# lukasmolnar/pino-locoman

Measured on AMD Instinct MI355X. Metric: MPC solves/sec (B2G whole_body_rnea N=50) at batch; 1/2/4/8 GPU, higher is better.
Workload: dtype f64; 1 GPU; b2g whole_body_rnea N=50 MPC step; batch_per_gpu=1024, global_batch=1024, nodes=50, robot=b2g, dynamics=whole_body_rnea, solver=osqp-sqp (1 SQP iteration, max_iter 100), parallelism=batch-sharded dp1

## Files before the change

include/pinoloco.h:

```cpp
#ifndef PINOLOCO_H_
#define PINOLOCO_H_

#ifdef __cplusplus
extern "C" {
#endif

typedef struct pl_model pl_model;
typedef struct pl_ocp pl_ocp;

#define PL_JOINT_FREEFLYER 1
#define PL_JOINT_REVOLUTE 2

#define PL_DYN_WHOLE_BODY_RNEA 0
#define PL_DYN_WHOLE_BODY_ACC 1
#define PL_DYN_WHOLE_BODY_ABA 2
#define PL_DYN_CENTROIDAL_VEL 3
#define PL_DYN_CENTROIDAL_ACC 4

typedef struct {
  int njoints;
  int nq, nv;
  const int* parent;
  const int* jtype;
  const double* axis;
// ... 194 lines not shown
int pl_dyn_jac_sizes(const pl_dyn* d, int fn, int flags, int* in_len, int* tan_len, int* out_len);
int pl_dyn_jac(pl_dyn* d, int fn, int batch, int frame, int flags, unsigned wrt, const double* in0,
               const double* in1, const double* in2, const double* in3, double* out, double* jac);
int pl_dyn_jac_device(pl_dyn* d, int fn, int batch, int frame, int flags, unsigned wrt, const void* in0,
                      const void* in1, const void* in2, const void* in3, void* out, void* jac);

#define PL_ADMM_AUTO 0
#define PL_ADMM_SWEEP 1
#define PL_ADMM_SWEEP2 2
#define PL_ADMM_CHAIN 3
int pl_ocp_set_admm_kernel(pl_ocp* o, int kind);
int pl_ocp_get_admm_kernel(const pl_ocp* o);
int pl_ocp_get_admm_groups(const pl_ocp* o);
#define PL_ADMM_OPERANDS_SPLIT 0
#define PL_ADMM_OPERANDS_FUSED 1
int pl_ocp_set_admm_operands(pl_ocp* o, int mode);
int pl_ocp_get_admm_operands(const pl_ocp* o);
int pl_ocp_get_admm_rho_from_bounds(const pl_ocp* o);

int pl_ocp_profile(pl_ocp* o, int enable);
int pl_ocp_profile_read(pl_ocp* o, double* out);
int pl_ocp_profile_read_hess(pl_ocp* o, double* out);
int pl_ocp_sizes(const pl_ocp* o, long long* out);

int pl_debug_get(pl_ocp* o, const char* name, double* out, long long count);
int pl_debug_set(pl_ocp* o, const char* name, const double* in, long long count);
int pl_debug_nodes(const pl_ocp* o, int* out);
int pl_debug_consts(const pl_ocp* o, void* model_out, void* oc_out, int* sizes);
int pl_debug_admm(pl_ocp* o, int niter, int reset);
int pl_debug_qp_setup(pl_ocp* o);
int pl_debug_check(pl_ocp* o, int final_check, int unscale);

#ifdef __cplusplus
}
#endif
#endif
```

pino-locoman_amd/csrc/api.hip:

```cpp
#include "api_internal.h"
#include "plant.h"
#include "record.h"
#include "retract.h"

#include <map>

static thread_local char g_err[1024] = "";

void pl_set_error(const char* fmt, ...) {
  va_list ap;
  va_start(ap, fmt);
  vsnprintf(g_err, sizeof(g_err), fmt, ap);
  va_end(ap);
}



extern "C" const char* pl_last_error(void) { return g_err; }
extern "C" int pl_version(void) { return 1; }

#ifndef PL_SRC_SHA
#define PL_SRC_SHA "unknown"
#endif
extern "C" const char* pl_build_info(void) { return "pl_src_sha256=" PL_SRC_SHA " arch=gfx950"; }
// ... 1658 lines not shown
  if (!out) { pl_set_error("null argument"); return -1; }
  prof_collect(&o->h);
  out[0] = o->h.prof_hess_ms;
  out[1] = (double)o->h.prof_hess_launches;
  int lanes = 0;
  if (o->h.d.ip_act)
    PL_CHECK_HIP(hipMemcpy(&lanes, o->h.d.ip_act + o->h.B + 1, sizeof(int), hipMemcpyDeviceToHost));
  out[2] = o->h.prof_hess_launches > 0 ? (double)lanes / o->h.prof_hess_launches : 0.0;
  return 0;
}

int admm_lds_bytes(const PlOcpHandle* h);
int admm_ppw(const PlOcpHandle* h);
int admm_asb_cap(const PlOcpHandle* h);

extern "C" int pl_ocp_sizes(const pl_ocp* o, long long* out) {
  if (!o) { pl_set_error("null handle"); return -1; }
  out[0] = o->h.n; out[1] = o->h.m; out[2] = o->h.nnz; out[3] = o->h.S_stride; out[4] = o->h.nw_max; out[5] = o->h.N;
  out[6] = (long long)o->aprog.size(); out[7] = admm_ppw(&o->h); out[8] = admm_lds_bytes(&o->h); out[9] = o->h.admm_asr;
  out[10] = admm_asb_cap(&o->h); out[11] = o->h.nent_max; out[12] = o->h.debug_paths;
  return 0;
}

static int debug_rw(pl_ocp* o, const char* name, double* out, const double* in, long long count) {
  PlOcpHandle* h = &o->h;
  const size_t B = h->B;
  struct Item { const char* n; double* p; size_t len; } items[] = {
      {"Hlag", h->d.Hlag, h->d.Hlag ? B * (size_t)h->hl_stride : 0},
      {"ip_dwi", h->d.ip_dwi, h->d.ip_dwi ? 2 * B : 0},
      {"As", h->d.As, B * h->nnz}, {"Araw", h->d.Araw, B * h->nnz}, {"qs", h->d.qs, B * h->n},
      {"ls", h->d.ls, B * h->m},   {"us", h->d.us, B * h->m},       {"rho", h->d.rho, B * h->m},
      {"D", h->d.D, B * h->n},     {"E", h->d.E, B * h->m},         {"cs", h->d.cs, B},
      {"admm_t", h->d.dbg, h->d.dbg ? B * 40 : 0}, {"Ps", h->d.Ps, B * h->n},   {"P", h->d.P, B * h->n},         {"xa", h->d.xa, B * h->n},
      {"za", h->d.za, B * h->m},   {"ya", h->d.ya, B * h->m},       {"S", h->d.S, B * (size_t)h->S_stride},
      {"FS", h->d.FS, h->d.FS ? B * (size_t)h->fs_stride : 0},
      {"rhs", h->d.rhs, B * h->n}, {"step", h->d.step, B * h->n},   {"grad", h->d.grad, B * h->n},
      {"g", h->d.g, B * h->m},     {"xstate", h->d.xstate, B * h->nx},
      {"dxs", h->d.dxs, B * h->n}, {"dys", h->d.dys, B * h->m},     {"chk", h->d.chk, B * (size_t)(h->N + 1) * 8},
      {"lbg", h->d.lbg, B * h->m}, {"ubg", h->d.ubg, B * h->m},
      {"rhoc", h->d.rhoc, B * (size_t)(h->N + 1) * std::max(h->ncpl_max, 1)},
      {"ip_s", h->d.ip_s, h->d.ip_s ? B * h->m : 0},     {"ip_lam", h->d.ip_lam, h->d.ip_lam ? B * h->m : 0},
      {"ip_lam0", h->d.ip_lam0, h->d.ip_lam0 ? B * h->m : 0},
      {"ip_zl", h->d.ip_zl, h->d.ip_zl ? B * h->m : 0},  {"ip_zu", h->d.ip_zu, h->d.ip_zu ? B * h->m : 0},
      {"ip_rh", h->d.ip_rh, h->d.ip_rh ? B * h->m : 0},  {"ip_dl", h->d.ip_dl, h->d.ip_dl ? B * h->m : 0},
      {"ip_ds", h->d.ip_ds, h->d.ip_ds ? B * h->m : 0},  {"ip_dx", h->d.ip_dx, h->d.ip_dx ? B * h->n : 0},
      {"ip_jdx", h->d.ip_jdx, h->d.ip_jdx ? B * h->m : 0}};
// ... 108 lines not shown
```

pino-locoman_amd/csrc/dyn_jac.h:

```cpp
#pragma once
#include "dyn.h"

namespace pl {

enum { PL_JF_NONE = -1, PL_JF_TREE = 0, PL_JF_COMP, PL_JF_ABA, PL_JF_CEN, PL_JF_FRAME, PL_JF_COUNT };

PL_HD int dyn_jac_family(int fn) {
  switch (fn) {
    case PL_FN_RNEA: case PL_FN_NLE: case PL_FN_GAPS_WB: return PL_JF_TREE;
    case PL_FN_GAPS_CA: case PL_FN_BASE_ACC_WB: case PL_FN_BASE_ACC_CV: return PL_JF_COMP;
    case PL_FN_ABA: return PL_JF_ABA;
    case PL_FN_COM_DYN: case PL_FN_GAPS_CV: case PL_FN_BASE_VEL_CV: case PL_FN_COM: return PL_JF_CEN;
    case PL_FN_FRAME_POS: case PL_FN_FRAME_VEL: return PL_JF_FRAME;
    default: return PL_JF_NONE;
  }
}
PL_HD int dyn_jac_cfg_input(int fn) { return (fn == PL_FN_BASE_VEL_CV || fn == PL_FN_GAPS_CV) ? 1 : 0; }
PL_HD void dyn_jac_tan_len(const PlModel& M, int fn, int nf, int* in_len, int* tan_len) {
  dyn_in_len(M, fn, nf, in_len);
  for (int k = 0; k < 4; ++k) tan_len[k] = in_len[k];
  tan_len[dyn_jac_cfg_input(fn)] = M.nv;
}
PL_HD void dyn_jac_locate(const int* tan_len, unsigned wrt, int col, int* input, int* local) {
  *input = -1;
// ... 107 lines not shown
    tree_pass<Dual>(M, O, qb, qr, SeedIn{in1, s1, 0}, SeedIn{nle ? nullptr : in2, s2, 0},
                    SeedIn{nle ? nullptr : in3, s3, 0}, true, false, kin);
    for (int r = 0; r < 6; ++r) out[r * ostride] = kin.tau[r].d;
    if (fn != PL_FN_GAPS_WB)
      for (int r = 6; r < nv; ++r) {
        const Dual t = kin.tau_j(r - 6);
        out[r * ostride] = t.d;
      }
  } else if constexpr (FAM == PL_JF_COMP) {
    Dual comp[15], res[6];
    const bool gap = fn == PL_FN_GAPS_CA;
    tree_pass<Dual>(M, O, qb, qr, SeedIn{in1, s1, 0}, SeedIn{in2, s2, gap ? 0 : 6}, SeedIn{in3, s3, 0}, true, false,
                    kin, comp, std::true_type{});
    if (gap) {
      centroidal_gap(M.total_mass, qb, comp, res);
    } else {
      Dual R0[9];
      quat_to_R(qb + 3, R0);
      base_solve(M.total_mass, R0, comp, kin.tau, res);
    }
    for (int r = 0; r < 6; ++r) out[r * ostride] = res[r].d;
  } else if constexpr (FAM == PL_JF_ABA) {
    tree_pass<Dual>(M, O, qb, qr, SeedIn{in1, s1, 0}, ShAcc{aba_sh}, SeedIn{in3, s3, 0}, true, false, kin);
    double* x = kin.dst + (PL_MAXV - 6 + 3 * PL_MAXFEET) * kin.dstride;
    for (int r = 0; r < 6; ++r) x[r * kin.dstride] = -kin.tau[r].d;
    for (int r = 0; r < nj; ++r) {
      const Dual t = kin.tau_j(r);
      x[(6 + r) * kin.dstride] = (r == s2 ? 1.0 : 0.0) - t.d;
    }
    chol_solve_strided(aba_sh + PL_MAXV, nv, x, kin.dstride);
    for (int r = 0; r < nv; ++r) out[r * ostride] = x[r * kin.dstride];
  } else if constexpr (FAM == PL_JF_CEN) {
    Dual hg[6], hd[6], ci[9];
    if (fn == PL_FN_COM_DYN) {
      centroidal_pass<Dual>(M, O, qb, qr, SeedIn{nullptr, -1, 0}, SeedIn{in1, s1, 0}, false, true, hg, hd);
      for (int r = 0; r < 6; ++r) out[r * ostride] = hd[r].d;
    } else if (fn == PL_FN_GAPS_CV) {
      centroidal_pass<Dual>(M, O, qb, qr, SeedIn{in2, s2, 0}, SeedIn{nullptr, -1, 0}, true, false, hg, hd);
      for (int r = 0; r < 6; ++r) out[r * ostride] = hg[r].d - (r == s0 ? M.total_mass : 0.0);
    } else if (fn == PL_FN_BASE_VEL_CV) {
      centroidal_pass<Dual>(M, O, qb, qr, SeedIn{in2, s2, 6}, SeedIn{nullptr, -1, 0}, true, false, hg, hd, ci,
                            std::true_type{});
      Dual R0[9], h[6], vb[6];
      quat_to_R(qb + 3, R0);
      for (int r = 0; r < 6; ++r) h[r] = Dual(in0[r], r == s0 ? 1.0 : 0.0);
      base_vel_solve(M.total_mass, R0, qb, ci, h, hg, vb);
      for (int r = 0; r < 6; ++r) out[r * ostride] = vb[r].d;
// ... 66 lines not shown
```

pino-locoman_amd/csrc/k_eval.hip:

```cpp
#include "dyn.h"
#include "eval_common.h"

using pl::VecIn;

namespace {

struct ValueEmit {
  double* g;
  double* lb;
  double* ub;
  int r;
  __device__ void operator()(double v, double l, double u) {
    g[r] = v;
    lb[r] = l;
    ub[r] = u;
    ++r;
  }
};

struct JacEmit {
  const int* rowidx;
  double* out;
  int ptr, end, r;
  __device__ void operator()(const Dual& v, double, double) {
// ... 23 lines not shown
template <int DYN>
__global__ __launch_bounds__(64) void k_eval_values(PlDev d, int B, int N, int n, int m, int np, const double* __restrict__ xsrc) {
  const int tid = blockIdx.x * blockDim.x + threadIdx.x;
  if (tid >= B * N) return;
  const int b = tid / N, i = tid - b * N;
  if (ip_skip(d, b)) return;
  const PlOcpConst& O = *d.oc;
  const PlModel& M = *d.model;
  const PlNode nd = d.nodes[i];
  const PlNode nn = d.nodes[i + 1];
  const double* x = xsrc + (size_t)b * n;
  const double* p = d.p + (size_t)b * np;
  VecIn<double> dx, u, dxn;
  node_inputs(d, nd, nn, x, nullptr, 0.0, -1, &dx, &u, &dxn, O.ndx);
  ValueEmit e{d.g + (size_t)b * m + nd.row_off, d.lbg + (size_t)b * m + nd.row_off,
              d.ubg + (size_t)b * m + nd.row_off, 0};
  __shared__ double kst[PL_KIN_STORE * 64];
  pl::node_rows<double, DYN>(M, O, i, p, dx, u, dxn, e, kst + threadIdx.x, 64);
}

#ifndef PL_JAC_WAVES
#define PL_JAC_WAVES 1
#endif
template <int DYN>
__global__ __launch_bounds__(64) __attribute__((amdgpu_waves_per_eu(PL_JAC_WAVES)))
void k_eval_jac(PlDev d, int B, int N, int n, int np, int nnz, int jl_len) {
  const int b = blockIdx.y;
  if (ip_skip(d, b)) return;
  const int q = (int)blockIdx.x * 64 + threadIdx.x;
  constexpr bool CH = DYN == PL_DYN_RNEA || DYN == PL_DYN_ACC;
  constexpr int SLOTS = CH ? PL_JAC_SLOTS_CH : PL_JAC_SLOTS;
  const int first = d.jlist[blockIdx.x * 64].x;
  const bool valid = q < jl_len && d.jlist[min(q, jl_len - 1)].x >= 0;
  const int2 jw = valid ? d.jlist[q] : make_int2(first, 0);
  const int i = jw.x, lc = jw.y & 0xffff, only_ch = CH ? (jw.y >> 16) - 1 : -1;
  const int slot = min(i - first, SLOTS - 1);
  __shared__ double kst_tan[PL_KIN_STORE_DUAL * 64];
  __shared__ double kst_val[SLOTS * PL_KIN_STORE_DUAL];
  double* aba_slot = nullptr;
  if constexpr (DYN == PL_DYN_ABA) {
    __shared__ double aba_sh[PL_JAC_SLOTS * PL_ABA_SH];
    aba_slot = aba_sh + slot * PL_ABA_SH;
    const int nv = d.oc->nv;
    double* raw = kst_tan + slot * ((PL_KIN_STORE_DUAL * 64) / PL_JAC_SLOTS);
    const bool tree = valid && lc < d.nodes[i].nw;
    int s0 = threadIdx.x, s1 = threadIdx.x;
    const int wb = (int)blockIdx.x * 64;
    if (tree) {
      while (s0 > 0 && d.jlist[wb + s0 - 1].x == i) --s0;
      while (s1 < 63 && wb + s1 + 1 < jl_len && d.jlist[wb + s1 + 1].x == i) ++s1;
    }
    const double* pb = d.p + (size_t)b * np;
    const double* dxi = d.x + (size_t)b * n + d.nodes[i].x_off;
    if (tree)
      for (int c = threadIdx.x - s0; c < nv + 2; c += s1 - s0 + 1) pl::aba_primal_column(*d.model, *d.oc, pb, dxi, c, raw + c * nv);
    __syncthreads();
    if (tree && threadIdx.x == s0) pl::aba_primal_finish(*d.oc, dxi, raw, aba_slot);
    __syncthreads();
  }
  if (!valid) return;
  const PlNode nd = d.nodes[i];
  const int* cp = d.colptr + nd.colptr_off;
  const int e0 = cp[lc], e1 = cp[lc + 1];
  const PlOcpConst& O = *d.oc;
  const PlModel& M = *d.model;
  const PlNode nn = d.nodes[i + 1];
  const double* x = d.x + (size_t)b * n;
  const double* p = d.p + (size_t)b * np;
  const int ndx = O.ndx;
  VecIn<Dual> dx{x + nd.x_off, nullptr, 0.0, lc};
  VecIn<Dual> u{x + nd.x_off + ndx, nullptr, 0.0, lc - ndx};
  VecIn<Dual> dxn{x + nn.x_off, nullptr, 0.0, lc - nd.nw};
  JacEmit e{d.rowidx + nd.ent_off, d.Araw + (size_t)b * nnz + nd.ent_off, e0, e1, 0};
  pl::node_rows<Dual, DYN>(M, O, i, p, dx, u, dxn, e, reinterpret_cast<Dual*>(kst_tan + threadIdx.x), 64,
                           kst_val + slot * PL_KIN_STORE_DUAL, aba_slot, nullptr, only_ch);
}

namespace {
struct ZeroInD {
  PL_HD double operator[](int) const { return 0.0; }
};
struct UnitIn {
  int k;
  PL_HD double operator[](int j) const { return j == k ? 1.0 : 0.0; }
};
}

template <int DYN>
__global__ __launch_bounds__(64) void k_eval_jac_lin(PlDev d, int B, int n, int np, int nnz, int len) {
  const int b = blockIdx.y;
  if (ip_skip(d, b)) return;
  const int q = (int)blockIdx.x * 64 + threadIdx.x;
  __shared__ double kst[PL_KIN_STORE * 64];
  __shared__ double kval[PL_KIN_STORE];
  for (int k = threadIdx.x; k < PL_KIN_STORE; k += 64) kval[k] = 0.0;
  __syncthreads();
  if (q >= len) return;
  const int2 jw = d.jlin[q];
// ... 4 lines not shown
  const PlNode nn = d.nodes[i + 1];
  const int ndx = O.ndx;
  const double* x = d.x + (size_t)b * n;
  const double* p = d.p + (size_t)b * np;
  const double* xi = p + O.P.x_init;
  const VecIn<double> dq{x + nd.x_off, nullptr, 0.0, -1};
  double qb[7];
  pl::integrate_ff<double>(xi, dq, qb);
  const pl::RevQ<double, VecIn<double>> qrev{xi, dq};
  pl::NodeKin<double> kp;
  kp.store = kst + threadIdx.x;
  kp.stride = 64;
  const int k = lc - ndx;
  pl::tree_pass<double>(*d.model0, O, qb, qrev, ZeroInD{}, UnitIn{k < O.na ? k : -1}, UnitIn{k - O.na}, true, false,
                        kp, nullptr, std::false_type{}, only_ch);
  double base[6];
  for (int r = 0; r < 6; ++r) base[r] = kp.tau[r];
  const int* cp = d.colptr + nd.colptr_off;
  VecIn<Dual> dx{x + nd.x_off, nullptr, 0.0, lc};
  VecIn<Dual> u{x + nd.x_off + ndx, nullptr, 0.0, lc - ndx};
  VecIn<Dual> dxn{x + nn.x_off, nullptr, 0.0, lc - nd.nw};
  JacEmit e{d.rowidx + nd.ent_off, d.Araw + (size_t)b * nnz + nd.ent_off, cp[lc], cp[lc + 1], 0};
  pl::node_rows<Dual, DYN>(*d.model, O, i, p, dx, u, dxn, e, reinterpret_cast<Dual*>(kst + threadIdx.x), 64, kval,
                           nullptr, base);
}

__global__ __launch_bounds__(256) void k_objective(PlDev d, int N, int n, int np) {
  const int b = blockIdx.x;
  if (ip_skip(d, b)) return;
  __shared__ double red[256];
  double f = objective_wg<true>(d, b, N, n, np, d.x + (size_t)b * n, nullptr, 0.0, d.grad + (size_t)b * n, red);
  if (threadIdx.x == 0) d.work[(size_t)b * 8 + 0] = f;
}

__global__ __launch_bounds__(256) void k_hess(PlDev d, int N, int n, int np) {
  const int b = blockIdx.x;
  const PlOcpConst& O = *d.oc;
  const double* p = d.p + (size_t)b * np;
  double* P = d.P + (size_t)b * n;
  for (int j = threadIdx.x; j < n; j += blockDim.x) {
    const int i = d.colnode[j];
    const int lc = j - d.nodes[i].x_off;
    double h;
    if (lc < O.ndx) {
      h = 2.0 * p[O.P.Q_diag + lc];
    } else {
      int k = lc - O.ndx;
// ... 3 lines not shown
    P[j] = h;
  }
}

#define PL_DISPATCH_DYN(dyn, KERNEL, ...)                                          \
  switch (dyn) {                                                                    \
    case PL_DYN_RNEA: hipLaunchKernelGGL(KERNEL<PL_DYN_RNEA>, __VA_ARGS__); break; \
    case PL_DYN_ACC: hipLaunchKernelGGL(KERNEL<PL_DYN_ACC>, __VA_ARGS__); break;   \
    case PL_DYN_CV: hipLaunchKernelGGL(KERNEL<PL_DYN_CV>, __VA_ARGS__); break;     \
    case PL_DYN_CA: hipLaunchKernelGGL(KERNEL<PL_DYN_CA>, __VA_ARGS__); break;     \
    case PL_DYN_ACCNB: hipLaunchKernelGGL(KERNEL<PL_DYN_ACCNB>, __VA_ARGS__); break; \
    case PL_DYN_CVNB: hipLaunchKernelGGL(KERNEL<PL_DYN_CVNB>, __VA_ARGS__); break;   \
    case PL_DYN_RNEAFD: hipLaunchKernelGGL(KERNEL<PL_DYN_RNEAFD>, __VA_ARGS__); break; \
    default: hipLaunchKernelGGL(KERNEL<PL_DYN_ABA>, __VA_ARGS__); break;           \
  }

void launch_eval_values(PlOcpHandle* h, const double* xsrc) {
  const int total = h->B * h->N;
  const int bs = 64;
  PL_DISPATCH_DYN(h->oc.dyn, k_eval_values, dim3((total + bs - 1) / bs), dim3(bs), 0, h->stream, h->d, h->B, h->N,
                  h->n, h->m, h->np, xsrc);
}

void launch_eval_jac(PlOcpHandle* h) {
  if (h->jlin_len > 0) {
    const dim3 g((h->jlin_len + 63) / 64, h->B);
    if (h->oc.dyn == PL_DYN_RNEA)
      hipLaunchKernelGGL(k_eval_jac_lin<PL_DYN_RNEA>, g, dim3(64), 0, h->stream, h->d, h->B, h->n, h->np, h->nnz,
                         h->jlin_len);
    else if (h->oc.dyn == PL_DYN_ACC)
      hipLaunchKernelGGL(k_eval_jac_lin<PL_DYN_ACC>, g, dim3(64), 0, h->stream, h->d, h->B, h->n, h->np, h->nnz,
                         h->jlin_len);
    else
      hipLaunchKernelGGL(k_eval_jac_lin<PL_DYN_RNEAFD>, g, dim3(64), 0, h->stream, h->d, h->B, h->n, h->np, h->nnz,
                         h->jlin_len);
  }
  const int len = (h->jac_cheap_ok && !h->jac_cheap_every) ? h->jl_ex : h->jl_len;
  if (len > 0)
    PL_DISPATCH_DYN(h->oc.dyn, k_eval_jac, dim3((len + 63) / 64, h->B), dim3(64), 0, h->stream, h->d, h->B, h->N,
                    h->n, h->np, h->nnz, h->jl_len);
  h->jac_cheap_ok = 1;
}

void launch_objective(PlOcpHandle* h) {
  hipLaunchKernelGGL(k_objective, dim3(h->B), dim3(256), 0, h->stream, h->d, h->N, h->n, h->np);
}

void launch_hess(PlOcpHandle* h) {
  hipLaunchKernelGGL(k_hess, dim3(h->B), dim3(256), 0, h->stream, h->d, h->N, h->n, h->np);
}

namespace {
struct ViolEmit {
  double ss, mx;
  __device__ void operator()(double v, double l, double u) {
    double a = fmax(0.0, l - v), c = fmax(0.0, v - u);
    ss += a * a + c * c;
    mx = fmax(mx, fmax(a, c));
  }
};

template <int DYN>
__device__ void violation_at(const PlDev& d, int b, int N, int n, int np, const double* x, const double* step,
                             double alpha, double* kst, double* red, double* metric, double* vmax) {
// ... 170 lines not shown
```

pino-locoman_amd/csrc/rbd.h:

```cpp
#pragma once
#include <type_traits>

#include "ad.h"
#include "model.h"

namespace pl {

template <class S> PL_HD void cross3(const S* a, const S* b, S* o) {
  S x = a[1] * b[2] - a[2] * b[1];
  S y = a[2] * b[0] - a[0] * b[2];
  S z = a[0] * b[1] - a[1] * b[0];
  o[0] = x; o[1] = y; o[2] = z;
}
template <class S> PL_HD S dot3(const S* a, const S* b) { return a[0] * b[0] + a[1] * b[1] + a[2] * b[2]; }
template <class S, class T, class X> PL_HD void matvec(const T* R, const X* x, S* o) {
  S a = R[0] * x[0] + R[1] * x[1] + R[2] * x[2];
  S b = R[3] * x[0] + R[4] * x[1] + R[5] * x[2];
  S c = R[6] * x[0] + R[7] * x[1] + R[8] * x[2];
  o[0] = a; o[1] = b; o[2] = c;
}
template <class S, class T, class X> PL_HD void mattvec(const T* R, const X* x, S* o) {
  S a = R[0] * x[0] + R[3] * x[1] + R[6] * x[2];
  S b = R[1] * x[0] + R[4] * x[1] + R[7] * x[2];
  S c = R[2] * x[0] + R[5] * x[1] + R[8] * x[2];
// ... 168 lines not shown
  S pxf[3];
  cross3(pp, fl, pxf);
  for (int k = 0; k < 3; ++k) { out[k] = fl[k]; out[3 + k] = nl[k] + pxf[k]; }
}
template <class S> PL_HD void inertia_mul(double m, const double* c, const double* Ic, const S* v, S* out) {
  S cc[3] = {S(c[0]), S(c[1]), S(c[2])};
  S cxw[3];
  cross3(cc, v + 3, cxw);
  S fl[3] = {m * (v[0] - cxw[0]), m * (v[1] - cxw[1]), m * (v[2] - cxw[2])};
  S Iw[3];
  matvec(Ic, v + 3, Iw);
  S cxf[3];
  cross3(cc, fl, cxf);
  for (int k = 0; k < 3; ++k) { out[k] = fl[k]; out[3 + k] = Iw[k] + cxf[k]; }
}
template <class S> PL_HD void motion_cross_force(const S* v, const S* f, S* out) {
  S a[3], b[3], c[3];
  cross3(v + 3, f, a);
  cross3(v + 3, f + 3, b);
  cross3(v, f, c);
  for (int k = 0; k < 3; ++k) { out[k] = a[k]; out[3 + k] = b[k] + c[k]; }
}

#define PL_KIN_STORE (PL_MAXV - 6 + 3 * PL_MAXFEET + 7 * PL_MAXCL)
#define PL_KIN_STORE_DUAL PL_KIN_STORE
#ifndef PL_CHAIN_UNROLL
#define PL_CHAIN_UNROLL 1
#endif
template <class S> struct NodeKin {
  S tau[6];
  S arm_vel[3];
  S* store;
  int stride;
  PL_HD S& tau_j(int k) { return store[k * stride]; }
  PL_HD S& foot_vel(int e, int c) { return store[(PL_MAXV - 6 + 3 * e + c) * stride]; }
  PL_HD S& sw(int kk, int c) { return store[(PL_MAXV - 6 + 3 * PL_MAXFEET + 7 * kk + c) * stride]; }
  PL_HD S& alpha(int kk) { return store[(PL_MAXV - 6 + 3 * PL_MAXFEET + 7 * kk + 6) * stride]; }
  PL_HD void clear(int k) { store[k * stride] = S(0.0); }
};

struct DualRef {
  double* v;
  double* d;
  PL_HD operator Dual() const { return Dual(*v, *d); }
  PL_HD DualRef& operator=(const Dual& x) {
    *v = x.v;
    *d = x.d;
    return *this;
  }
};
template <> struct NodeKin<Dual> {
  Dual tau[6];
  Dual arm_vel[3];
  double* vst;
  double* dst;
  int vstride, dstride;
  PL_HD DualRef at(int k) { return DualRef{vst + k * vstride, dst + k * dstride}; }
  PL_HD DualRef tau_j(int k) { return at(k); }
  PL_HD DualRef foot_vel(int e, int c) { return at(PL_MAXV - 6 + 3 * e + c); }
  PL_HD DualRef sw(int kk, int c) { return at(PL_MAXV - 6 + 3 * PL_MAXFEET + 7 * kk + c); }
  PL_HD DualRef alpha(int kk) { return at(PL_MAXV - 6 + 3 * PL_MAXFEET + 7 * kk + 6); }
  PL_HD void clear(int k) { dst[k * dstride] = 0.0; }
};

template <class S, class In> struct RevQ {
  const double* q0;
  In dq;
  PL_HD S operator()(int k) const { return q0[k] + dq[k - 1]; }
};
template <class S, class In> struct VelAcc {
  const double* v0;
  In dv;
  PL_HD S operator[](int k) const { return v0[k] + dv[k]; }
};
template <class S> struct RevQArr {
  const S* q;
  PL_HD S operator()(int k) const { return q[k]; }
};

template <class S>
PL_HD void comp_add(S* comp, double m, const double* lever, const double* Ic, const S* oR, const S* op, const S* p0) {
  S lw[3];
  matvec(oR, lever, lw);
  S r[3];
// ... 656 lines not shown
```

pino-locoman_amd/csrc/rows.h:

```cpp
#pragma once
#include <type_traits>

#include "rbd.h"

namespace pl {

PL_HD double spline_vel_z(double phase, double period, double h_max, double v_lo, double v_td) {
  double mid = period / 2.0;
  double t = phase * period;
  double t0, dt, c1, c2, c3;
  if (phase < 0.5) {
    t0 = 0.0; dt = mid - 0.0;
    double p0 = 0.0, v0 = v_lo, p1 = h_max, v1 = 0.0;
    double dpos = p1 - p0, dvel = v1 - v0;
    c1 = v0 * dt; c2 = -(3.0 * v0 + dvel) * dt + 3.0 * dpos; c3 = (2.0 * v0 + dvel) * dt - 2.0 * dpos;
  } else {
    t0 = mid; dt = period - mid;
    double p0 = h_max, v0 = 0.0, p1 = 0.0, v1 = v_td;
    double dpos = p1 - p0, dvel = v1 - v0;
    c1 = v0 * dt; c2 = -(3.0 * v0 + dvel) * dt + 3.0 * dpos; c3 = (2.0 * v0 + dvel) * dt - 2.0 * dpos;
  }
  double tn = (t - t0) / dt;
  return (3.0 * c3 * tn * tn + 2.0 * c2 * tn + c1) / dt;
}
// ... 71 lines not shown
PL_HD void chol_solve(const double* L, int n, double* x) {
  for (int i = 0; i < n; ++i) {
    const double* Li = L + i * (i + 1) / 2;
    double t = x[i];
    for (int k = 0; k < i; ++k) t -= Li[k] * x[k];
    x[i] = t / Li[i];
  }
  for (int i = n - 1; i >= 0; --i) {
    double t = x[i];
    for (int k = i + 1; k < n; ++k) t -= L[k * (k + 1) / 2 + i] * x[k];
    x[i] = t / L[i * (i + 1) / 2 + i];
  }
}

template <class E>
PL_HD auto emit_skip(E& e, int n, int) -> decltype(e.skip_block(n)) { return e.skip_block(n); }
template <class E>
PL_HD bool emit_skip(E&, int, long) { return false; }

template <class S, int DYN, class Emit>
PL_HD void node_rows(const PlModel& M, const PlOcpConst& O, int i, const double* p, const VecIn<S>& dx,
                     const VecIn<S>& u, const VecIn<S>& dxn, Emit& emit, S* kstore, int kstride,
                     double* kvals = nullptr, const double* aba_sh = nullptr, const double* lin_base = nullptr,
                     int only_ch = -1) {
  const int nv = O.nv, nq = O.nq, nj = O.nj;
  constexpr bool CV = PL_IS_CV(DYN);
  constexpr bool CVNB = (DYN == PL_DYN_CVNB);
  const double* xi = p + O.P.x_init;
  const double dt = node_dt(O, p, i);
  const int type = node_type(O, i);
  const double* xq = CV ? xi + 6 : xi;
  const VecIn<S> dq = CV ? sub_in(dx, 6) : dx;
  S qb[7];
  integrate_ff<S>(xq, dq, qb);
  const RevQ<S, VecIn<S>> qrev{xq, dq};
  S vnb[CVNB ? PL_MAXV : 1], hdot_nb[CVNB ? 6 : 1];
  if constexpr (CVNB) {
    bool run = true;
    if constexpr (!std::is_same<S, double>::value) run = !seeded(dxn, 0, O.ndx);
    if (run) {
      S hj[6], ci[9], hcur[6], R0[9];
      centroidal_pass<S>(M, O, qb, qrev, ZeroBaseAcc<S>{u}, sub_in(u, nj), true, true, hj, hdot_nb, ci,
                         std::true_type{});
      for (int k = 0; k < 6; ++k) hcur[k] = xi[k] + dx[k];
      quat_to_R(qb + 3, R0);
      base_vel_solve(M.total_mass, R0, qb, ci, hcur, hj, vnb);
    } else {
      for (int k = 0; k < 6; ++k) { vnb[k] = S(0.0); hdot_nb[k] = S(0.0); }
    }
    for (int k = 0; k < nj; ++k) vnb[6 + k] = u[k];
  }
  const auto vel = [&]() {
    if constexpr (CVNB) return static_cast<const S*>(vnb);
    else if constexpr (CV) return u;
    else return VelAcc<S, VecIn<S>>{xi + nq, sub_in(dx, nv)};
  }();
  constexpr bool ACCF = (DYN == PL_DYN_ACC || DYN == PL_DYN_CA || DYN == PL_DYN_ACCNB);
  constexpr bool NB = (DYN == PL_DYN_ACCNB);
  constexpr bool COMP = (DYN == PL_DYN_CA || DYN == PL_DYN_ACCNB);
  constexpr bool FD = (DYN == PL_DYN_RNEAFD);
  const int f_off = (PL_IS_RNEA(DYN) || ACCF) ? O.na : (DYN == PL_DYN_CV ? nv : nj);
  const VecIn<S> a = u;
  const FdAcc<S> afd{xi + nq, sub_in(dx, nv), sub_in(dxn, nv), dt};
  const VecIn<S> forces = sub_in(u, f_off);
  const VecIn<S> tau_j = sub_in(u, PL_IS_RNEA(DYN) ? O.na + O.nf : 0);
  const bool state_rows = CV || (type != 0);
  NodeKin<S> kin;
  if constexpr (std::is_same<S, Dual>::value) {
    double* raw = reinterpret_cast<double*>(kstore);
    if (kvals) {
      kin.vst = kvals;
      kin.vstride = 1;
      kin.dst = raw;
      kin.dstride = kstride;
    } else {
      kin.vst = raw;
      kin.dst = raw + 1;
      kin.vstride = kin.dstride = 2 * kstride;
    }
  } else {
    (void)kvals;
    kin.store = kstore;
    kin.stride = kstride;
  }
  constexpr bool want_tau = (PL_IS_RNEA(DYN) || ACCF);
  bool tree = true, cen = CV;
  if constexpr (!std::is_same<S, double>::value) {
    const bool seed_dxn = seeded(dxn, 0, FD ? nv : O.ndx);
    const bool seed_tau = PL_IS_RNEA(DYN) && seeded(u, O.na + O.nf, O.na + O.nf + nj);
    const bool seed_h = DYN == PL_DYN_CV && seeded(dx, 0, 6);
    const bool seed_f = CV && seeded(u, f_off, f_off + O.nf);
    const bool seed_pos = (PL_IS_RNEA(DYN) || DYN == PL_DYN_ACC) && seeded(dx, 0, 3);
    tree = !(seed_dxn || seed_tau || seed_h || seed_f || seed_pos) && !lin_base;
    cen = DYN == PL_DYN_CV && !(seed_dxn || seed_h);
  } else {
    (void)lin_base;
  }
  S comp[COMP ? 15 : 1];
  S aba_a[DYN == PL_DYN_ABA ? PL_MAXV : 1];
  bool aba_done = false;
  if constexpr (DYN == PL_DYN_ABA && std::is_same<S, Dual>::value) {
    {
      if (tree) {
        tree_pass<S>(M, O, qb, qrev, vel, ShAcc{aba_sh}, forces, true, state_rows, kin);
        double r[PL_MAXV];
        for (int k = 0; k < 6; ++k) r[k] = -kin.tau[k].d;
        for (int k = 0; k < nj; ++k) {
          const Dual t = kin.tau_j(k);
          r[6 + k] = tau_j[k].d - t.d;
        }
        chol_solve(aba_sh + PL_MAXV, nv, r);
        for (int k = 0; k < nv; ++k) aba_a[k] = Dual(aba_sh[k], r[k]);
      } else {
        for (int k = 0; k < PL_KIN_STORE_DUAL; ++k) kin.clear(k);
        for (int k = 0; k < 3; ++k) kin.arm_vel[k] = S(0.0);
        for (int k = 0; k < nv; ++k) aba_a[k] = S(0.0);
      }
      aba_done = true;
    }
  }
  if (aba_done) {
  } else if (tree && (want_tau || state_rows)) {
    if constexpr (NB) {
      tree_pass<S>(M, O, qb, qrev, vel, ZeroBaseAcc<S>{a}, forces, want_tau, state_rows, kin, comp, std::true_type{});
    } else if constexpr (COMP) {
      tree_pass<S>(M, O, qb, qrev, vel, a, forces, want_tau, state_rows, kin, comp, std::true_type{});
    } else if constexpr (FD) {
      tree_pass<S>(M, O, qb, qrev, vel, afd, forces, want_tau, state_rows, kin, nullptr, std::false_type{}, only_ch);
    } else {
      tree_pass<S>(M, O, qb, qrev, vel, a, forces, want_tau, state_rows, kin, nullptr, std::false_type{}, only_ch);
    }
  } else {
    for (int k = lin_base ? nj : 0; k < PL_KIN_STORE_DUAL; ++k) kin.clear(k);
    for (int k = 0; k < 3; ++k) kin.arm_vel[k] = S(0.0);
    for (int k = 0; k < 6; ++k) kin.tau[k] = S(0.0);
    if constexpr (COMP)
      for (int k = 0; k < 15; ++k) comp[k] = S(0.0);
    if constexpr (std::is_same<S, Dual>::value)
      if (lin_base)
        for (int k = 0; k < 6; ++k) kin.tau[k] = Dual(0.0, lin_base[k]);
  }
  S abase[NB ? 6 : 1], cgap[DYN == PL_DYN_CA ? 6 : 1];
  if constexpr (COMP) {
    if (tree) {
      S R0[9];
      quat_to_R(qb + 3, R0);
      if constexpr (NB) base_solve(M.total_mass, R0, comp, kin.tau, abase);
      else centroidal_gap(M.total_mass, qb, comp, cgap);
    } else {
      for (int k = 0; k < 6; ++k) {
        if constexpr (NB) abase[k] = S(0.0);
        else cgap[k] = S(0.0);
      }
    }
  }
  S hg[CV ? 6 : 1], hdot[CV ? 6 : 1];
// ... 111 lines not shown
```

pino-locoman_amd/pinoloco/_lib.py:

```python
from __future__ import annotations

import ctypes as C
import os

import numpy as np

HERE = os.path.dirname(os.path.abspath(__file__))
LIB_PATH = os.environ.get("PINOLOCO_LIB") or os.path.join(HERE, "libpinoloco.so")

_dp = C.POINTER(C.c_double)
_ip = C.POINTER(C.c_int)


class ModelDesc(C.Structure):
    _fields_ = [("njoints", C.c_int), ("nq", C.c_int), ("nv", C.c_int),
                ("parent", _ip), ("jtype", _ip), ("axis", _dp), ("placement_R", _dp), ("placement_p", _dp),
                ("mass", _dp), ("lever", _dp), ("inertia", _dp), ("gravity", _dp),
                ("nframes", C.c_int), ("frame_parent", _ip), ("frame_R", _dp), ("frame_p", _dp)]


class OcpDesc(C.Structure):
    _fields_ = [("dynamics", C.c_int), ("nodes", C.c_int), ("tau_nodes", C.c_int), ("include_acc", C.c_int),
                ("include_base", C.c_int), ("n_feet", C.c_int), ("foot_frames", C.c_int * 4),
                ("ext_force_frame", C.c_int), ("arm_ee_frame", C.c_int), ("base_frame", C.c_int),
# ... 93 lines not shown
    "pl_mpc_download": (C.c_int, [C.c_void_p, _dp]),
    "pl_ocp_retract_sizes": (C.c_int, [C.c_void_p, C.c_int, C.c_int, C.POINTER(C.c_longlong)]),
    "pl_ocp_retract": (C.c_int, [C.c_void_p, C.c_int, C.c_int, _dp, _dp, _dp, _dp, _dp, _dp]),
    "pl_ocp_retract_device": (C.c_int, [C.c_void_p, C.c_int, C.c_int, C.c_void_p]),
    "pl_ocp_profile_read_hess": (C.c_int, [C.c_void_p, _dp]),
    "pl_mpc_graph_info": (C.c_int, [C.c_void_p, C.POINTER(C.c_longlong)]),
    "pl_mpc_set_ip_lam": (C.c_int, [C.c_void_p, C.c_int]),
    "pl_mpc_log_start": (C.c_int, [C.c_void_p, C.c_longlong, C.c_int, _dp, _dp]),
    "pl_mpc_log_stop": (C.c_int, [C.c_void_p]),
    "pl_mpc_log_sizes": (C.c_int, [C.c_void_p, _llp]),
    "pl_mpc_log_read": (C.c_int, [C.c_void_p, C.c_longlong, C.c_longlong, _dp]),
    "pl_mpc_log_device": (C.c_int, [C.c_void_p, C.POINTER(C.c_void_p)]),
    "pl_mpc_metrics": (C.c_int, [C.c_void_p, C.POINTER(MpcMetrics)]),
    "pl_mpc_record_host": (C.c_int, [C.c_void_p, C.c_int, _dp, _dp, C.POINTER(Stats), _dp, _dp, _dp, C.c_double,
                                     _dp, _dp, _llp, _dp, C.POINTER(MpcMetrics)]),
    "pl_mpc_set_push": (C.c_int, [C.c_void_p, _ip, _ip, _dp]),
    "pl_mpc_run": (C.c_int, [C.c_void_p, C.c_int, C.c_int]),
    "pl_ocp_sync": (C.c_int, [C.c_void_p]),
    "pl_state_integrate": (C.c_int, [C.c_void_p, _dp, _dp, _dp]),
    "pl_state_difference": (C.c_int, [C.c_void_p, _dp, _dp, _dp]),
    "pl_ocp_profile": (C.c_int, [C.c_void_p, C.c_int]),
    "pl_ocp_profile_read": (C.c_int, [C.c_void_p, _dp]),
    "pl_ocp_sizes": (C.c_int, [C.c_void_p, C.POINTER(C.c_longlong)]),
    "pl_debug_consts": (C.c_int, [C.c_void_p, C.c_void_p, C.c_void_p, _ip]),
    "pl_debug_get": (C.c_int, [C.c_void_p, C.c_char_p, _dp, C.c_longlong]),
    "pl_debug_set": (C.c_int, [C.c_void_p, C.c_char_p, _dp, C.c_longlong]),
    "pl_debug_nodes": (C.c_int, [C.c_void_p, _ip]),
    "pl_debug_admm": (C.c_int, [C.c_void_p, C.c_int, C.c_int]),
    "pl_debug_qp_setup": (C.c_int, [C.c_void_p]),
    "pl_debug_check": (C.c_int, [C.c_void_p, C.c_int, C.c_int]),
    "pl_dyn_create": (C.c_int, [C.c_void_p, _ip, C.c_int, C.c_int, C.c_int, C.POINTER(C.c_void_p)]),
    "pl_dyn_destroy": (None, [C.c_void_p]),
    "pl_dyn_sizes": (C.c_int, [C.c_void_p, C.c_int, C.c_int, _ip, _ip]),
    "pl_dyn_eval": (C.c_int, [C.c_void_p, C.c_int, C.c_int, C.c_int, C.c_int, _dp, _dp, _dp, _dp, _dp]),
    "pl_dyn_jac_sizes": (C.c_int, [C.c_void_p, C.c_int, C.c_int, _ip, _ip, _ip]),
    "pl_dyn_jac": (C.c_int, [C.c_void_p, C.c_int, C.c_int, C.c_int, C.c_int, C.c_uint, _dp, _dp, _dp, _dp, _dp, _dp]),
    "pl_dyn_jac_device": (C.c_int, [C.c_void_p, C.c_int, C.c_int, C.c_int, C.c_int, C.c_uint, C.c_void_p, C.c_void_p,
                                    C.c_void_p, C.c_void_p, C.c_void_p, C.c_void_p]),
}

_lib = None


class PinolocoError(RuntimeError):
    pass

# ... 95 lines not shown
```

pino-locoman_amd/pinoloco/ocp.py:

```python
from __future__ import annotations

import ctypes as C
import time

import numpy as np

from . import _lib
from .dynamics import DYNAMICS_CLASSES, Dynamics
from .gait import horizon_dts

DYN_CODES = {"whole_body_rnea": 0, "whole_body_acc": 1, "whole_body_aba": 2, "centroidal_vel": 3,
             "centroidal_acc": 4}
GAIT_CODES = {"trot": 0, "walk": 1, "stand": 2}
SOLVER_CODES = {"osqp": 0, "fatrop": 1}

OSQP_SETTINGS = dict(max_iter=100, alpha=1.4, rho=2e-2, warm_start=True, adaptive_rho=False,
                     sigma=1e-6, eps_abs=1e-3, eps_rel=1e-3, eps_prim_inf=1e-4, eps_dual_inf=1e-4,
                     scaling=10, check_termination=25)

FATROP_SETTINGS = dict(max_iter=10, tol=1e-3, mu_init=1e-4, bound_push=1e-7, bound_frac=1e-2, delta_w=1e-8,
                       delta_c=1e-4, ls_max=12, n_refine=8, hessian=0)
IP_HESSIAN = {"exact": 0, "gauss_newton": 1}

OCP_ARGS = {
# ... 591 lines not shown
        return {"captures": int(out[0]), "replays": int(out[1]), "eager_fallback": int(out[2])}

    def sync(self):
        _lib.check(_lib.lib().pl_ocp_sync(self.h))

    def profile(self, enable):
        _lib.check(_lib.lib().pl_ocp_profile(self.h, int(enable)))

    def profile_read(self):
        out = np.zeros(3)
        _lib.check(_lib.lib().pl_ocp_profile_read(self.h, _lib.dptr(out)))
        return {"admm_ms": out[0], "launches": int(out[1]), "problem_iters": int(out[2])}

    def profile_read_hess(self):
        out = np.zeros(3)
        _lib.check(_lib.lib().pl_ocp_profile_read_hess(self.h, _lib.dptr(out)))
        return {"hess_ms": out[0], "launches": int(out[1]), "lanes": out[2]}

    def sizes(self):
        out = (C.c_longlong * 13)()
        _lib.check(_lib.lib().pl_ocp_sizes(self.h, out))
        return dict(zip(("n", "m", "nnz", "S_stride", "nw_max", "N", "admm_prog", "admm_ppw", "admm_lds_bytes",
                         "admm_asr", "admm_asb_cap", "nent_max", "debug_paths"), [int(v) for v in out]))

    def close(self):
        if getattr(self, "h", None):
            _lib.lib().pl_ocp_destroy(self.h)
            self.h = None

    def __del__(self):
        try:
            self.close()
        except Exception:
            pass


class ModelCache:
    _cache = {}

    @classmethod
    def get(cls, model):
        key = id(model)
        if key not in cls._cache:
            cls._cache[key] = (model, _lib.ModelHandle(model))
        return cls._cache[key][1]

# ... 382 lines not shown
```

Measured before the change: 10210 solves/s.

## Shrink k_eval_jac LDS footprint via dynamic shared memory and scratch sink layout

Reorders the kinematic store so foot-velocity and contact scratch come first and tau last. The Jacobian kernel's value store now keeps only the per-slot non-scratch part and sends output values to a shared sink. For RNEA/ACC the LDS is allocated dynamically, sized by the model's actual joint count instead of PL_MAXV. The smaller LDS use is meant to allow more resident waves per CU. It also adds an API to report LDS sizes, and the index remapping risks subtle aliasing bugs.

```diff
diff --git a/include/pinoloco.h b/include/pinoloco.h
--- a/include/pinoloco.h
+++ b/include/pinoloco.h
@@ -240,6 +240,8 @@
 int pl_ocp_profile_read(pl_ocp* o, double* out);
 int pl_ocp_profile_read_hess(pl_ocp* o, double* out);
 int pl_ocp_sizes(const pl_ocp* o, long long* out);
+#define PL_LDS_SIZES_LEN 50
+int pl_ocp_lds_sizes(const pl_ocp* o, long long* out);
 
 int pl_debug_get(pl_ocp* o, const char* name, double* out, long long count);
 int pl_debug_set(pl_ocp* o, const char* name, const double* in, long long count);
diff --git a/pino-locoman_amd/csrc/api.hip b/pino-locoman_amd/csrc/api.hip
--- a/pino-locoman_amd/csrc/api.hip
+++ b/pino-locoman_amd/csrc/api.hip
@@ -1704,6 +1704,23 @@
   return 0;
 }
 
+int eval_jac_lds_bytes(const PlOcpHandle* h, int* out);
+
+extern "C" int pl_ocp_lds_sizes(const pl_ocp* o, long long* out) {
+  if (!o || !out) { pl_set_error("null argument"); return -1; }
+  int jac = 0;
+  if (eval_jac_lds_bytes(&o->h, &jac) != 0) { pl_set_error("hipFuncGetAttributes(k_eval_jac) failed"); return -1; }
+  out[0] = jac;
+  out[1] = o->h.nfgroup;
+  for (int g = 0; g < PL_FAC_MAXGROUPS; ++g) {
+    const bool on = g < o->h.nfgroup;
+    out[2 + 3 * g] = on ? o->h.fg_i0[g] : 0;
+    out[3 + 3 * g] = on ? o->h.fg_n[g] : 0;
+    out[4 + 3 * g] = on ? o->h.fg_lds[g] : 0;
+  }
+  return 0;
+}
+
 static int debug_rw(pl_ocp* o, const char* name, double* out, const double* in, long long count) {
   PlOcpHandle* h = &o->h;
   const size_t B = h->B;
diff --git a/pino-locoman_amd/csrc/dyn_jac.h b/pino-locoman_amd/csrc/dyn_jac.h
--- a/pino-locoman_amd/csrc/dyn_jac.h
+++ b/pino-locoman_amd/csrc/dyn_jac.h
@@ -153,7 +153,7 @@
     for (int r = 0; r < 6; ++r) out[r * ostride] = res[r].d;
   } else if constexpr (FAM == PL_JF_ABA) {
     tree_pass<Dual>(M, O, qb, qr, SeedIn{in1, s1, 0}, ShAcc{aba_sh}, SeedIn{in3, s3, 0}, true, false, kin);
-    double* x = kin.dst + (PL_MAXV - 6 + 3 * PL_MAXFEET) * kin.dstride;
+    double* x = kin.dst + PL_KIN_SCR * kin.dstride;
     for (int r = 0; r < 6; ++r) x[r * kin.dstride] = -kin.tau[r].d;
     for (int r = 0; r < nj; ++r) {
       const Dual t = kin.tau_j(r);
diff --git a/pino-locoman_amd/csrc/k_eval.hip b/pino-locoman_amd/csrc/k_eval.hip
--- a/pino-locoman_amd/csrc/k_eval.hip
+++ b/pino-locoman_amd/csrc/k_eval.hip
@@ -69,6 +69,14 @@
 #ifndef PL_JAC_WAVES
 #define PL_JAC_WAVES 1
 #endif
+#define PL_JAC_LDS_BUDGET 40960
+constexpr int jac_val_doubles(int slots) { return (slots * PL_KIN_NSCR + 2) & ~1; }
+constexpr int jac_lds_bytes(int slots, int nj) { return (jac_val_doubles(slots) + (PL_KIN_TAU + nj) * 64) * 8; }
+static_assert(jac_lds_bytes(PL_JAC_SLOTS_CH, 18) <= PL_JAC_LDS_BUDGET,
+              "k_eval_jac<RNEA / ACC>: a wave of an 18-joint model must fit a quarter of the CU's LDS");
+static_assert(jac_lds_bytes(PL_JAC_SLOTS, PL_MAXV - 6) <= PL_JAC_LDS_BUDGET,
+              "k_eval_jac, three-slot instantiations: the store must fit a quarter of the CU's LDS");
+extern __shared__ double jac_dyn_lds[];
 template <int DYN>
 __global__ __launch_bounds__(64) __attribute__((amdgpu_waves_per_eu(PL_JAC_WAVES)))
 void k_eval_jac(PlDev d, int B, int N, int n, int np, int nnz, int jl_len) {
@@ -82,8 +90,16 @@
   const int2 jw = valid ? d.jlist[q] : make_int2(first, 0);
   const int i = jw.x, lc = jw.y & 0xffff, only_ch = CH ? (jw.y >> 16) - 1 : -1;
   const int slot = min(i - first, SLOTS - 1);
-  __shared__ double kst_tan[PL_KIN_STORE_DUAL * 64];
-  __shared__ double kst_val[SLOTS * PL_KIN_STORE_DUAL];
+  double *kst_tan, *kst_val;
+  if constexpr (CH) {
+    kst_val = jac_dyn_lds;
+    kst_tan = jac_dyn_lds + jac_val_doubles(SLOTS);
+  } else {
+    __shared__ double tan_st[PL_KIN_STORE_DUAL * 64];
+    __shared__ double val_st[jac_val_doubles(SLOTS)];
+    kst_tan = tan_st;
+    kst_val = val_st;
+  }
   double* aba_slot = nullptr;
   if constexpr (DYN == PL_DYN_ABA) {
     __shared__ double aba_sh[PL_JAC_SLOTS * PL_ABA_SH];
@@ -120,7 +136,7 @@
   VecIn<Dual> dxn{x + nn.x_off, nullptr, 0.0, lc - nd.nw};
   JacEmit e{d.rowidx + nd.ent_off, d.Araw + (size_t)b * nnz + nd.ent_off, e0, e1, 0};
   pl::node_rows<Dual, DYN>(M, O, i, p, dx, u, dxn, e, reinterpret_cast<Dual*>(kst_tan + threadIdx.x), 64,
-                           kst_val + slot * PL_KIN_STORE_DUAL, aba_slot, nullptr, only_ch);
+                           kst_val + slot * PL_KIN_NSCR, aba_slot, nullptr, only_ch, kst_val + SLOTS * PL_KIN_NSCR);
 }
 
 namespace {
@@ -171,7 +187,7 @@
   VecIn<Dual> dxn{x + nn.x_off, nullptr, 0.0, lc - nd.nw};
   JacEmit e{d.rowidx + nd.ent_off, d.Araw + (size_t)b * nnz + nd.ent_off, cp[lc], cp[lc + 1], 0};
   pl::node_rows<Dual, DYN>(*d.model, O, i, p, dx, u, dxn, e, reinterpret_cast<Dual*>(kst + threadIdx.x), 64, kval,
-                           nullptr, base);
+                           nullptr, base, -1, kval + PL_KIN_NSCR);
 }
 
 __global__ __launch_bounds__(256) void k_objective(PlDev d, int N, int n, int np) {
@@ -221,6 +237,11 @@
                   h->n, h->m, h->np, xsrc);
 }
 
+static int jac_dynamic_lds(const PlOcpHandle* h) {
+  const bool ch = h->oc.dyn == PL_DYN_RNEA || h->oc.dyn == PL_DYN_ACC;
+  return ch ? jac_lds_bytes(PL_JAC_SLOTS_CH, h->oc.nj) : 0;
+}
+
 void launch_eval_jac(PlOcpHandle* h) {
   if (h->jlin_len > 0) {
     const dim3 g((h->jlin_len + 63) / 64, h->B);
@@ -236,9 +257,27 @@
   }
   const int len = (h->jac_cheap_ok && !h->jac_cheap_every) ? h->jl_ex : h->jl_len;
   if (len > 0)
-    PL_DISPATCH_DYN(h->oc.dyn, k_eval_jac, dim3((len + 63) / 64, h->B), dim3(64), 0, h->stream, h->d, h->B, h->N,
-                    h->n, h->np, h->nnz, h->jl_len);
+    PL_DISPATCH_DYN(h->oc.dyn, k_eval_jac, dim3((len + 63) / 64, h->B), dim3(64), jac_dynamic_lds(h), h->stream, h->d,
+                    h->B, h->N, h->n, h->np, h->nnz, h->jl_len);
   h->jac_cheap_ok = 1;
+}
+
+int eval_jac_lds_bytes(const PlOcpHandle* h, int* out) {
+  hipFuncAttributes a;
+  hipError_t e;
+  switch (h->oc.dyn) {
+    case PL_DYN_RNEA: e = hipFuncGetAttributes(&a, reinterpret_cast<const void*>(&k_eval_jac<PL_DYN_RNEA>)); break;
+    case PL_DYN_ACC: e = hipFuncGetAttributes(&a, reinterpret_cast<const void*>(&k_eval_jac<PL_DYN_ACC>)); break;
+    case PL_DYN_CV: e = hipFuncGetAttributes(&a, reinterpret_cast<const void*>(&k_eval_jac<PL_DYN_CV>)); break;
+    case PL_DYN_CA: e = hipFuncGetAttributes(&a, reinterpret_cast<const void*>(&k_eval_jac<PL_DYN_CA>)); break;
+    case PL_DYN_ACCNB: e = hipFuncGetAttributes(&a, reinterpret_cast<const void*>(&k_eval_jac<PL_DYN_ACCNB>)); break;
+    case PL_DYN_CVNB: e = hipFuncGetAttributes(&a, reinterpret_cast<const void*>(&k_eval_jac<PL_DYN_CVNB>)); break;
+    case PL_DYN_RNEAFD: e = hipFuncGetAttributes(&a, reinterpret_cast<const void*>(&k_eval_jac<PL_DYN_RNEAFD>)); break;
+    default: e = hipFuncGetAttributes(&a, reinterpret_cast<const void*>(&k_eval_jac<PL_DYN_ABA>)); break;
+  }
+  if (e != hipSuccess) return -1;
+  *out = (int)a.sharedSizeBytes + jac_dynamic_lds(h);
+  return 0;
 }
 
 void launch_objective(PlOcpHandle* h) {
diff --git a/pino-locoman_amd/csrc/rbd.h b/pino-locoman_amd/csrc/rbd.h
--- a/pino-locoman_amd/csrc/rbd.h
+++ b/pino-locoman_amd/csrc/rbd.h
@@ -214,7 +214,10 @@
   for (int k = 0; k < 3; ++k) { out[k] = a[k]; out[3 + k] = b[k] + c[k]; }
 }
 
-#define PL_KIN_STORE (PL_MAXV - 6 + 3 * PL_MAXFEET + 7 * PL_MAXCL)
+#define PL_KIN_SCR (3 * PL_MAXFEET)
+#define PL_KIN_NSCR (7 * PL_MAXCL)
+#define PL_KIN_TAU (PL_KIN_SCR + PL_KIN_NSCR)
+#define PL_KIN_STORE (PL_KIN_TAU + PL_MAXV - 6)
 #define PL_KIN_STORE_DUAL PL_KIN_STORE
 #ifndef PL_CHAIN_UNROLL
 #define PL_CHAIN_UNROLL 1
@@ -224,10 +227,10 @@
   S arm_vel[3];
   S* store;
   int stride;
-  PL_HD S& tau_j(int k) { return store[k * stride]; }
-  PL_HD S& foot_vel(int e, int c) { return store[(PL_MAXV - 6 + 3 * e + c) * stride]; }
-  PL_HD S& sw(int kk, int c) { return store[(PL_MAXV - 6 + 3 * PL_MAXFEET + 7 * kk + c) * stride]; }
-  PL_HD S& alpha(int kk) { return store[(PL_MAXV - 6 + 3 * PL_MAXFEET + 7 * kk + 6) * stride]; }
+  PL_HD S& tau_j(int k) { return store[(PL_KIN_TAU + k) * stride]; }
+  PL_HD S& foot_vel(int e, int c) { return store[(3 * e + c) * stride]; }
+  PL_HD S& sw(int kk, int c) { return store[(PL_KIN_SCR + 7 * kk + c) * stride]; }
+  PL_HD S& alpha(int kk) { return store[(PL_KIN_SCR + 7 * kk + 6) * stride]; }
   PL_HD void clear(int k) { store[k * stride] = S(0.0); }
 };
 
@@ -247,11 +250,23 @@
   double* vst;
   double* dst;
   int vstride, dstride;
-  PL_HD DualRef at(int k) { return DualRef{vst + k * vstride, dst + k * dstride}; }
-  PL_HD DualRef tau_j(int k) { return at(k); }
-  PL_HD DualRef foot_vel(int e, int c) { return at(PL_MAXV - 6 + 3 * e + c); }
-  PL_HD DualRef sw(int kk, int c) { return at(PL_MAXV - 6 + 3 * PL_MAXFEET + 7 * kk + c); }
-  PL_HD DualRef alpha(int kk) { return at(PL_MAXV - 6 + 3 * PL_MAXFEET + 7 * kk + 6); }
+  int omask = -1, soff = 0;
+  PL_HD void bind_scratch(double* scr, double* sink, double* d, int ds) {
+    vst = sink;
+    vstride = 1;
+    omask = 0;
+    soff = (int)(scr - sink) - PL_KIN_SCR;
+    dst = d;
+    dstride = ds;
+  }
+  PL_HD DualRef out_at(int k) { return DualRef{vst + (k & omask) * vstride, dst + k * dstride}; }
+  PL_HD DualRef scr_at(int k) {
+    return DualRef{vst + ((PL_KIN_SCR + k) * vstride + soff), dst + (PL_KIN_SCR + k) * dstride};
+  }
+  PL_HD DualRef tau_j(int k) { return out_at(PL_KIN_TAU + k); }
+  PL_HD DualRef foot_vel(int e, int c) { return out_at(3 * e + c); }
+  PL_HD DualRef sw(int kk, int c) { return scr_at(7 * kk + c); }
+  PL_HD DualRef alpha(int kk) { return scr_at(7 * kk + 6); }
   PL_HD void clear(int k) { dst[k * dstride] = 0.0; }
 };
 
diff --git a/pino-locoman_amd/csrc/rows.h b/pino-locoman_amd/csrc/rows.h
--- a/pino-locoman_amd/csrc/rows.h
+++ b/pino-locoman_amd/csrc/rows.h
@@ -117,7 +117,7 @@
 PL_HD void node_rows(const PlModel& M, const PlOcpConst& O, int i, const double* p, const VecIn<S>& dx,
                      const VecIn<S>& u, const VecIn<S>& dxn, Emit& emit, S* kstore, int kstride,
                      double* kvals = nullptr, const double* aba_sh = nullptr, const double* lin_base = nullptr,
-                     int only_ch = -1) {
+                     int only_ch = -1, double* ksink = nullptr) {
   const int nv = O.nv, nq = O.nq, nj = O.nj;
   constexpr bool CV = PL_IS_CV(DYN);
   constexpr bool CVNB = (DYN == PL_DYN_CVNB);
@@ -164,10 +164,7 @@
   if constexpr (std::is_same<S, Dual>::value) {
     double* raw = reinterpret_cast<double*>(kstore);
     if (kvals) {
-      kin.vst = kvals;
-      kin.vstride = 1;
-      kin.dst = raw;
-      kin.dstride = kstride;
+      kin.bind_scratch(kvals, ksink, raw, kstride);
     } else {
       kin.vst = raw;
       kin.dst = raw + 1;
@@ -207,7 +204,7 @@
         chol_solve(aba_sh + PL_MAXV, nv, r);
         for (int k = 0; k < nv; ++k) aba_a[k] = Dual(aba_sh[k], r[k]);
       } else {
-        for (int k = 0; k < PL_KIN_STORE_DUAL; ++k) kin.clear(k);
+        for (int k = 0; k < PL_KIN_TAU + nj; ++k) kin.clear(k);
         for (int k = 0; k < 3; ++k) kin.arm_vel[k] = S(0.0);
         for (int k = 0; k < nv; ++k) aba_a[k] = S(0.0);
       }
@@ -226,7 +223,7 @@
       tree_pass<S>(M, O, qb, qrev, vel, a, forces, want_tau, state_rows, kin, nullptr, std::false_type{}, only_ch);
     }
   } else {
-    for (int k = lin_base ? nj : 0; k < PL_KIN_STORE_DUAL; ++k) kin.clear(k);
+    for (int k = 0; k < (lin_base ? PL_KIN_TAU : PL_KIN_TAU + nj); ++k) kin.clear(k);
     for (int k = 0; k < 3; ++k) kin.arm_vel[k] = S(0.0);
     for (int k = 0; k < 6; ++k) kin.tau[k] = S(0.0);
     if constexpr (COMP)
diff --git a/pino-locoman_amd/pinoloco/_lib.py b/pino-locoman_amd/pinoloco/_lib.py
--- a/pino-locoman_amd/pinoloco/_lib.py
+++ b/pino-locoman_amd/pinoloco/_lib.py
@@ -139,6 +139,7 @@
     "pl_ocp_profile": (C.c_int, [C.c_void_p, C.c_int]),
     "pl_ocp_profile_read": (C.c_int, [C.c_void_p, _dp]),
     "pl_ocp_sizes": (C.c_int, [C.c_void_p, C.POINTER(C.c_longlong)]),
+    "pl_ocp_lds_sizes": (C.c_int, [C.c_void_p, C.POINTER(C.c_longlong)]),
     "pl_debug_consts": (C.c_int, [C.c_void_p, C.c_void_p, C.c_void_p, _ip]),
     "pl_debug_get": (C.c_int, [C.c_void_p, C.c_char_p, _dp, C.c_longlong]),
     "pl_debug_set": (C.c_int, [C.c_void_p, C.c_char_p, _dp, C.c_longlong]),
diff --git a/pino-locoman_amd/pinoloco/ocp.py b/pino-locoman_amd/pinoloco/ocp.py
--- a/pino-locoman_amd/pinoloco/ocp.py
+++ b/pino-locoman_amd/pinoloco/ocp.py
@@ -637,6 +637,12 @@
         _lib.check(_lib.lib().pl_ocp_sizes(self.h, out))
         return dict(zip(("n", "m", "nnz", "S_stride", "nw_max", "N", "admm_prog", "admm_ppw", "admm_lds_bytes",
                          "admm_asr", "admm_asb_cap", "nent_max", "debug_paths"), [int(v) for v in out]))
+
+    def lds_sizes(self):
+        out = (C.c_longlong * 50)()
+        _lib.check(_lib.lib().pl_ocp_lds_sizes(self.h, out))
+        groups = [tuple(int(v) for v in out[2 + 3 * g:5 + 3 * g]) for g in range(int(out[1]))]
+        return {"k_eval_jac": int(out[0]), "k_fnode": groups}
 
     def close(self):
         if getattr(self, "h", None):
```

Measured after the change: 10030 solves/s. -1.7%, worse.
